# hiimmuc/SpeakerVerification

Hardware: AMD Instinct MI355X
Metric: embeddings/sec (2 s @16 kHz) (higher is better)
Workload: dtype bf16

## Files before the change

### speakerverification_amd/csrc/res2net.hip

```cpp
#include "common.h"
#include "kernels.h"

namespace svhip {

namespace {

#ifdef SVHIP_GEMM_DEBUG
constexpr bool R2DBG = true;
#else
constexpr bool R2DBG = false;
#endif
constexpr int R2_TMAX = 416;

template <int CW, int MIT> struct R2Cfg {
    static constexpr int ROWB = CW * 2;
    static constexpr int NCH = ROWB / 16;
    static constexpr int NT = CW / 32;
    static constexpr int MW = 8 / NT;
    static constexpr int MI = MIT;
    static constexpr int TMAX = MW * MI * 32 < R2_TMAX ? MW * MI * 32 : R2_TMAX;
    static constexpr int U_BYTES = TMAX * ROWB;
    static constexpr int W_BYTES = CW * ROWB;
    static constexpr int LDS = U_BYTES + W_BYTES;
    static constexpr int WCH = CW * NCH / 512;
    static __device__ __forceinline__ int swz(int row) { return CW == 128 ? (row & 15) : ((row >> 1) & 7); }
};

template <int CW, int MIT>
__global__ __launch_bounds__(512, 2) void res2net_chain_kernel(Res2Params p) {
    typedef R2Cfg<CW, MIT> CF;
    constexpr int ROWB = CF::ROWB, NCH = CF::NCH, MI = CF::MI, WCH = CF::WCH;
    extern __shared__ __attribute__((aligned(16))) char smem[];
    char* U = smem;
    char* Wt = smem + CF::U_BYTES;

    const int S = p.slices > 1 ? p.slices : 1;
    const int b = (int)blockIdx.x / S, si = (int)blockIdx.x - b * S;
    const int Tg = p.T;
    const int c0 = S > 1 ? si * p.Tc : 0, c1 = S > 1 ? min(Tg, c0 + p.Tc) : Tg;
    const int l0 = S > 1 ? max(0, c0 - 7 * p.dil) : 0, l1 = S > 1 ? min(Tg, c1 + 7 * p.dil) : Tg;
    const int T = l1 - l0;
    const int tid = threadIdx.x, lane = tid & 63;
    const int wave = __builtin_amdgcn_readfirstlane(tid >> 6);
    const int wn = wave % CF::NT, wq = wave / CF::NT;
    const int fr = lane & 31, fh = lane >> 5;
    const bf16_t* __restrict__ H1 = reinterpret_cast<const bf16_t*>(p.H1) + ((int64_t)b * Tg + l0) * p.ld;
    bf16_t* __restrict__ H2 = reinterpret_cast<bf16_t*>(p.H2) + ((int64_t)b * Tg + l0) * p.ld;
    const int s0 = c0 - l0, s1 = c1 - l0;

    u32x4 wregs[WCH];
    auto wload = [&](int layer, int tap) {
        const char* wsrc = reinterpret_cast<const char*>(p.W[layer]);
        int tid_w = tid;
        asm volatile("" : "+v"(tid_w));
#pragma unroll
        for (int e = 0; e < WCH; ++e) {
            const int c = tid_w + 512 * e;
            const int n = c / NCH, ch = c % NCH;
            wregs[e] = *reinterpret_cast<const u32x4*>(wsrc + ((int64_t)n * p.Kp + tap * CW) * 2 + ch * 16);
        }
    };
    auto wstore = [&]() {
        int tid_w = tid;
        asm volatile("" : "+v"(tid_w));
#pragma unroll
        for (int e = 0; e < WCH; ++e) {
            const int c = tid_w + 512 * e;
            const int n = c / NCH, ch = c % NCH;
            *reinterpret_cast<u32x4*>(Wt + n * ROWB + ((ch ^ CF::swz(n)) << 4)) = wregs[e];
        }
    };

    wload(0, 0);
    {
        constexpr int RSTEP = 512 / NCH, RB0 = 4;
        const int row0 = tid / NCH, ch0 = tid % NCH;
        const uint32_t goff0 = ((uint32_t)row0 * (uint32_t)p.ld + (uint32_t)ch0 * 8u) * 2u;
        const uint32_t gstep = (uint32_t)RSTEP * (uint32_t)p.ld * 2u;
        const char* h1b = reinterpret_cast<const char*>(H1);
        char* h2b = reinterpret_cast<char*>(H2);
        for (int it0 = 0; it0 * RSTEP < T; it0 += RB0) {
            u32x4 cc0[RB0], cc1[RB0];
#pragma unroll
            for (int k = 0; k < RB0; ++k)
                if (row0 + (it0 + k) * RSTEP < T) {
                    cc0[k] = __builtin_nontemporal_load(reinterpret_cast<const u32x4*>(h1b + goff0 + (uint32_t)(it0 + k) * gstep));
                    cc1[k] = __builtin_nontemporal_load(reinterpret_cast<const u32x4*>(h1b + CW * 2 + goff0 + (uint32_t)(it0 + k) * gstep));
                }
#pragma unroll
            for (int k = 0; k < RB0; ++k) {
                const int row = row0 + (it0 + k) * RSTEP;
                if (row < T) {
                    if (row >= s0 && row < s1) *reinterpret_cast<u32x4*>(h2b + goff0 + (uint32_t)(it0 + k) * gstep) = cc0[k];
                    *reinterpret_cast<u32x4*>(U + row * ROWB + ((ch0 ^ CF::swz(row)) << 4)) = cc1[k];
                }
            }
        }
    }
    wstore();
    __syncthreads();
    const bool stamp = R2DBG && (p.debug & 64) && p.ts && tid == 0;
    unsigned long long tprev = 0;
    if (R2DBG && (p.debug & 64) && p.ts) tprev = __builtin_readcyclecounter();
    if (stamp) p.ts[(size_t)blockIdx.x * 32 + 3] = tprev;
#define R2_STAMP(stage, k) if (R2DBG && (p.debug & 64) && p.ts) { const unsigned long long t_ = __builtin_readcyclecounter(); if (stamp) p.ts[(size_t)blockIdx.x * 32 + (stage) * 4 + (k)] = t_ - tprev; tprev = t_; }

    for (int s = 1; s < 8; ++s) {
        const int layer = s - 1;
        f32x16 acc[MI];
        float zero = 0.0f;
        asm volatile("" : "+v"(zero));
#pragma unroll
        for (int i = 0; i < MI; ++i)
#pragma unroll
            for (int r = 0; r < 16; ++r) acc[i][r] = zero;

        constexpr int RSTEP = 512 / NCH;
        constexpr int RB = 7;
        constexpr int NPRE = (CF::TMAX / RSTEP + RB - 1) / RB * RB;
        const bool noglob = R2DBG && (p.debug & 1);

        u32x4 cpre[NPRE];
        for (int tap = 0; tap < 3; ++tap) {
            if (tap == 2 && s < 7 && !noglob) {
                int tid_p = tid;
                asm volatile("" : "+v"(tid_p));
                const int row0 = tid_p / NCH, ch0 = tid_p % NCH;
                const char* h1s = reinterpret_cast<const char*>(H1) + (s + 1) * CW * 2;
#pragma unroll
                for (int k = 0; k < NPRE; ++k) {
                    const int rowc = min(row0 + k * RSTEP, T - 1);
                    cpre[k] = __builtin_nontemporal_load(reinterpret_cast<const u32x4*>(h1s + ((uint32_t)rowc * (uint32_t)p.ld + (uint32_t)ch0 * 8u) * 2u));
                }
            }
            const bool more = !(s == 7 && tap == 2);
            if (more && !(R2DBG && (p.debug & 4))) { if (tap < 2) wload(layer, tap + 1); else wload(layer + 1, 0); }
            const int delta = (tap - 1) * p.dil;
            int fh_t = fh, fr_t = fr;
            asm volatile("" : "+v"(fh_t), "+v"(fr_t));
            int rbase[MI], rsw[MI];
#pragma unroll
            for (int i = 0; i < MI; ++i) {
                const int t = (wq + CF::MW * i) * 32 + fr_t + delta;
                const int row = min(max(reflect_idx(l0 + t, Tg) - l0, 0), T - 1);
                rbase[i] = row * ROWB;
                rsw[i] = CF::swz(row);
            }
            const int wrow = (wn * 32 + fr_t);
            const int wbase = wrow * ROWB, wsw = CF::swz(wrow);
            if (!(R2DBG && (p.debug & 2))) {
                constexpr int NK = CW / 16;
#pragma unroll
                for (int kk = 0; kk < NK; ++kk) {
                    const int ch = 2 * kk + fh_t;
                    const bf16x8 wf = *reinterpret_cast<const bf16x8*>(Wt + wbase + ((ch ^ wsw) << 4));
                    bf16x8 xf[MI];
#pragma unroll
                    for (int i = 0; i < MI; ++i) xf[i] = *reinterpret_cast<const bf16x8*>(U + rbase[i] + ((ch ^ rsw[i]) << 4));
#pragma unroll
                    for (int i = 0; i < MI; ++i) acc[i] = __builtin_amdgcn_mfma_f32_32x32x16_bf16(wf, xf[i], acc[i], 0, 0, 0);
                }
            }
            __syncthreads();
            if (tap < 2) { if (!(R2DBG && (p.debug & 4))) wstore(); __syncthreads(); }
        }

        R2_STAMP(s, 0)
        int fh_e = fh, fr_e = fr;
        asm volatile("" : "+v"(fh_e), "+v"(fr_e));
        if (!(R2DBG && (p.debug & 8)))
#pragma unroll
        for (int g = 0; g < 4; ++g) {
            const int n = wn * 32 + 8 * g + 4 * fh_e;
            const f32x4 b4 = *reinterpret_cast<const f32x4*>(p.bias[layer] + n);
            const f32x4 sc4 = *reinterpret_cast<const f32x4*>(p.scale[layer] + n);
            const f32x4 sh4 = *reinterpret_cast<const f32x4*>(p.shift[layer] + n);
#pragma unroll
            for (int i = 0; i < MI; ++i) {
                const int t = (wq + CF::MW * i) * 32 + fr_e;
                if (t < T) {
                    typedef bf16_t bf16x4 __attribute__((ext_vector_type(4)));
                    bf16x4 o;
#pragma unroll
                    for (int e = 0; e < 4; ++e) o[e] = static_cast<bf16_t>(fmaf(fmaxf(acc[i][4 * g + e] + b4[e], 0.0f), sc4[e], sh4[e]));
                    const int c8 = n >> 2;
                    *reinterpret_cast<bf16x4*>(U + t * ROWB + ((((c8 >> 1) ^ CF::swz(t)) << 4) | ((c8 & 1) << 3))) = o;
                }
            }
        }
        if (s < 7 && !(R2DBG && (p.debug & 4))) wstore();
        __syncthreads();
        R2_STAMP(s, 1)

        if (R2DBG && (p.debug & 32)) {
            for (int c = tid; c < T * NCH; c += 512) {
                const int row = c / NCH, ch = c % NCH;
                char* up = U + row * ROWB + ((ch ^ CF::swz(row)) << 4);
                const bf16x8 y = *reinterpret_cast<const bf16x8*>(up);
                if (row >= s0 && row < s1) *reinterpret_cast<bf16x8*>(H2 + (int64_t)row * p.ld + s * CW + ch * 8) = y;
                if (s < 7) {
                    const bf16x8 cn = *reinterpret_cast<const bf16x8*>(H1 + (int64_t)row * p.ld + (s + 1) * CW + ch * 8);
                    bf16x8 u;
#pragma unroll
                    for (int e = 0; e < 8; ++e) u[e] = static_cast<bf16_t>(static_cast<float>(y[e]) + static_cast<float>(cn[e]));
                    *reinterpret_cast<bf16x8*>(up) = u;
                }
            }
        } else {
            int tid_r = tid;
            asm volatile("" : "+v"(tid_r));
            const int row0 = tid_r / NCH, ch0 = tid_r % NCH;
            const uint32_t goff0 = ((uint32_t)row0 * (uint32_t)p.ld + (uint32_t)ch0 * 8u) * 2u;
            const uint32_t gstep = (uint32_t)RSTEP * (uint32_t)p.ld * 2u;
            char* h2s = reinterpret_cast<char*>(H2) + s * CW * 2;
#pragma unroll
            for (int g = 0; g < NPRE / RB; ++g) {
                const int it0 = g * RB;
                if (it0 * RSTEP < T) {
#pragma unroll
                    for (int k = 0; k < RB; ++k) {
                        const int row = row0 + (it0 + k) * RSTEP;
                        if (row < T) {
                            char* up = U + row * ROWB + ((ch0 ^ CF::swz(row)) << 4);
                            const bf16x8 y = *reinterpret_cast<const bf16x8*>(up);
                            if (!noglob && row >= s0 && row < s1) *reinterpret_cast<bf16x8*>(h2s + goff0 + (uint32_t)(it0 + k) * gstep) = y;
                            if (s < 7 && !noglob) {
                                const bf16x8 cv = __builtin_bit_cast(bf16x8, cpre[it0 + k]);
                                bf16x8 u;
#pragma unroll
                                for (int e = 0; e < 8; ++e) u[e] = static_cast<bf16_t>(static_cast<float>(y[e]) + static_cast<float>(cv[e]));
                                *reinterpret_cast<bf16x8*>(up) = u;
                            }
                        }
                    }
                }
            }
        }
        __syncthreads();
        R2_STAMP(s, 2)
    }
#undef R2_STAMP
}

template <int CW, int MIT>
hipError_t launch_cw(const Res2Params& p, int grid, hipStream_t stream) {
    static DeviceOnce attr;
    constexpr int lds = R2Cfg<CW, MIT>::LDS;
    if (hipError_t e = set_max_dynamic_lds(attr, reinterpret_cast<const void*>(res2net_chain_kernel<CW, MIT>), lds)) return e;
    hipLaunchKernelGGL((res2net_chain_kernel<CW, MIT>), dim3(grid), dim3(512), lds, stream, p);
    return hipGetLastError();
}

}

int res2net_chain_slices(int B, int C, int T, int dil, int num_cu) {
    const int cw = C / 8;
    const int tmax_s = cw == 128 ? R2Cfg<128, 3>::TMAX : R2Cfg<64, 2>::TMAX;
    int best = 1;
    for (int S = 2; S <= 7; ++S) {
        const int tc = (T + S - 1) / S;
        if ((int64_t)S * B > (int64_t)num_cu) break;
        if (tc + 14 * dil <= tmax_s && tc > 14 * dil) best = S;
    }
    return best;
}

bool res2net_chain_supported(int C, int T, int dil, int Kp) {
    const int cw = C / 8;
    return (cw == 64 || cw == 128) && T <= R2_TMAX && T > 2 * dil && Kp == 3 * cw;
}

hipError_t launch_res2net_chain(const Res2Params& p_in, int B, int C, hipStream_t stream) {
    if (!res2net_chain_supported(C, p_in.T, p_in.dil, p_in.Kp) || B <= 0 || p_in.ld % 8 != 0) return hipErrorInvalidValue;
    Res2Params p = p_in;
    if (p.slices > 1) {
        const int tmax_s = C / 8 == 128 ? R2Cfg<128, 3>::TMAX : R2Cfg<64, 2>::TMAX;
        while (p.slices > 1) {
            p.Tc = (p.T + p.slices - 1) / p.slices;
            if (p.Tc + 14 * p.dil <= tmax_s && p.Tc > 14 * p.dil) break;
            --p.slices;
        }
        if (p.slices > 1) return C / 8 == 128 ? launch_cw<128, 3>(p, B * p.slices, stream) : launch_cw<64, 2>(p, B * p.slices, stream);
    }
    p.slices = 1;
    return C / 8 == 128 ? launch_cw<128, 7>(p, B, stream) : launch_cw<64, 4>(p, B, stream);
}

}
```

Baseline: 60290.

## Add dedicated loader waves to res2net chain kernel for global I/O overlap

For the CW=128 non-sliced path, the kernel now launches 768 threads: 8 waves run the MFMA matmuls and 4 extra loader waves prefetch the next slice input from H1, add it into the LDS tile, and write finished outputs to H2. Global loads and stores are meant to overlap with compute instead of sitting serially between layers. The loader waves stay in lockstep with the compute waves through matching __syncthreads counts. The price is more threads per block, a lower occupancy bound of 3, and fragile barrier pairing between the two branches.

```diff
diff --git a/speakerverification_amd/csrc/res2net.hip b/speakerverification_amd/csrc/res2net.hip
--- a/speakerverification_amd/csrc/res2net.hip
+++ b/speakerverification_amd/csrc/res2net.hip
@@ -26,10 +26,10 @@
     static __device__ __forceinline__ int swz(int row) { return CW == 128 ? (row & 15) : ((row >> 1) & 7); }
 };
 
-template <int CW, int MIT>
-__global__ __launch_bounds__(512, 2) void res2net_chain_kernel(Res2Params p) {
+template <int CW, int MIT, bool LW>
+__global__ __launch_bounds__(LW ? 768 : 512, LW ? 3 : 2) void res2net_chain_kernel(Res2Params p) {
     typedef R2Cfg<CW, MIT> CF;
-    constexpr int ROWB = CF::ROWB, NCH = CF::NCH, MI = CF::MI, WCH = CF::WCH;
+    constexpr int ROWB = CF::ROWB, NCH = CF::NCH, MI = CF::MI;
     extern __shared__ __attribute__((aligned(16))) char smem[];
     char* U = smem;
     char* Wt = smem + CF::U_BYTES;
@@ -42,36 +42,68 @@
     const int T = l1 - l0;
     const int tid = threadIdx.x, lane = tid & 63;
     const int wave = __builtin_amdgcn_readfirstlane(tid >> 6);
+    const bool mat = !LW || wave < 8;
     const int wn = wave % CF::NT, wq = wave / CF::NT;
     const int fr = lane & 31, fh = lane >> 5;
     const bf16_t* __restrict__ H1 = reinterpret_cast<const bf16_t*>(p.H1) + ((int64_t)b * Tg + l0) * p.ld;
     bf16_t* __restrict__ H2 = reinterpret_cast<bf16_t*>(p.H2) + ((int64_t)b * Tg + l0) * p.ld;
     const int s0 = c0 - l0, s1 = c1 - l0;
 
+    constexpr int WT = 512;
+    constexpr int WCH = CW * NCH / WT;
+    const int wtid = tid;
     u32x4 wregs[WCH];
     auto wload = [&](int layer, int tap) {
         const char* wsrc = reinterpret_cast<const char*>(p.W[layer]);
-        int tid_w = tid;
+        int tid_w = wtid;
         asm volatile("" : "+v"(tid_w));
 #pragma unroll
         for (int e = 0; e < WCH; ++e) {
-            const int c = tid_w + 512 * e;
+            const int c = tid_w + WT * e;
             const int n = c / NCH, ch = c % NCH;
             wregs[e] = *reinterpret_cast<const u32x4*>(wsrc + ((int64_t)n * p.Kp + tap * CW) * 2 + ch * 16);
         }
     };
     auto wstore = [&]() {
-        int tid_w = tid;
+        int tid_w = wtid;
         asm volatile("" : "+v"(tid_w));
 #pragma unroll
         for (int e = 0; e < WCH; ++e) {
-            const int c = tid_w + 512 * e;
+            const int c = tid_w + WT * e;
             const int n = c / NCH, ch = c % NCH;
             *reinterpret_cast<u32x4*>(Wt + n * ROWB + ((ch ^ CF::swz(n)) << 4)) = wregs[e];
         }
     };
 
-    wload(0, 0);
+    constexpr int LROWS = 256 / NCH;
+    constexpr int NLC = LW ? (CF::TMAX + LROWS - 1) / LROWS : 1;
+    static_assert(!LW || (CW == 128 && NLC * LROWS <= CF::TMAX), "the loader rows cover U exactly");
+    u32x4 creg[NLC];
+    const int lt = LW ? tid - 512 : 0;
+    const int lrow0 = lt / NCH, lch = lt % NCH;
+    auto cload = [&](int sn) {
+        const char* h1s = reinterpret_cast<const char*>(H1) + sn * CW * 2;
+        int r0 = lrow0, c16 = lch * 16;
+        asm volatile("" : "+v"(r0), "+v"(c16));
+#pragma unroll
+        for (int k = 0; k < NLC; ++k) {
+            const int rowc = min(r0 + k * LROWS, T - 1);
+            creg[k] = __builtin_nontemporal_load(reinterpret_cast<const u32x4*>(h1s + ((uint32_t)rowc * (uint32_t)p.ld * 2u + (uint32_t)c16)));
+        }
+    };
+    auto ystore = [&](int sy) {
+        char* h2s = reinterpret_cast<char*>(H2) + sy * CW * 2;
+        int r0 = lrow0, c16 = lch * 16;
+        asm volatile("" : "+v"(r0), "+v"(c16));
+#pragma unroll
+        for (int k = 0; k < NLC; ++k) {
+            const int row = r0 + k * LROWS;
+            if (row < T) *reinterpret_cast<u32x4*>(h2s + ((uint32_t)row * (uint32_t)p.ld * 2u + (uint32_t)c16)) = creg[k];
+        }
+    };
+
+    if (mat) wload(0, 0);
+    if (mat)
     {
         constexpr int RSTEP = 512 / NCH, RB0 = 4;
         const int row0 = tid / NCH, ch0 = tid % NCH;
@@ -97,13 +129,122 @@
             }
         }
     }
-    wstore();
+    if (mat) wstore();
     __syncthreads();
     const bool stamp = R2DBG && (p.debug & 64) && p.ts && tid == 0;
     unsigned long long tprev = 0;
     if (R2DBG && (p.debug & 64) && p.ts) tprev = __builtin_readcyclecounter();
     if (stamp) p.ts[(size_t)blockIdx.x * 32 + 3] = tprev;
 #define R2_STAMP(stage, k) if (R2DBG && (p.debug & 64) && p.ts) { const unsigned long long t_ = __builtin_readcyclecounter(); if (stamp) p.ts[(size_t)blockIdx.x * 32 + (stage) * 4 + (k)] = t_ - tprev; tprev = t_; }
+
+    if constexpr (LW) {
+        const bool noglob = R2DBG && (p.debug & 1);
+        const bool noslab = R2DBG && (p.debug & 4);
+        if (mat) {
+            for (int s = 1; s < 8; ++s) {
+                const int layer = s - 1;
+                f32x16 acc[MI];
+                float zero = 0.0f;
+                asm volatile("" : "+v"(zero));
+#pragma unroll
+                for (int i = 0; i < MI; ++i)
+#pragma unroll
+                    for (int r = 0; r < 16; ++r) acc[i][r] = zero;
+                for (int tap = 0; tap < 3; ++tap) {
+                    if (!(s == 7 && tap == 2) && !noslab) { if (tap < 2) wload(layer, tap + 1); else wload(layer + 1, 0); }
+                    const int delta = (tap - 1) * p.dil;
+                    int fh_t = fh, fr_t = fr;
+                    asm volatile("" : "+v"(fh_t), "+v"(fr_t));
+                    int rbase[MI], rsw[MI];
+#pragma unroll
+                    for (int i = 0; i < MI; ++i) {
+                        const int t = (wq + CF::MW * i) * 32 + fr_t + delta;
+                        const int row = min(max(reflect_idx(t, Tg), 0), T - 1);
+                        rbase[i] = row * ROWB;
+                        rsw[i] = CF::swz(row);
+                    }
+                    const int wrow = (wn * 32 + fr_t);
+                    const int wbase = wrow * ROWB, wsw = CF::swz(wrow);
+                    if (!(R2DBG && (p.debug & 2))) {
+                        constexpr int NK = CW / 16;
+#pragma unroll
+                        for (int kk = 0; kk < NK; ++kk) {
+                            const int ch = 2 * kk + fh_t;
+                            const bf16x8 wf = *reinterpret_cast<const bf16x8*>(Wt + wbase + ((ch ^ wsw) << 4));
+                            bf16x8 xf[MI];
+#pragma unroll
+                            for (int i = 0; i < MI; ++i) xf[i] = *reinterpret_cast<const bf16x8*>(U + rbase[i] + ((ch ^ rsw[i]) << 4));
+#pragma unroll
+                            for (int i = 0; i < MI; ++i) acc[i] = __builtin_amdgcn_mfma_f32_32x32x16_bf16(wf, xf[i], acc[i], 0, 0, 0);
+                        }
+                    }
+                    __syncthreads();
+                    if (tap < 2) { if (!noslab) wstore(); __syncthreads(); }
+                }
+                R2_STAMP(s, 0)
+                int fh_e = fh, fr_e = fr;
+                asm volatile("" : "+v"(fh_e), "+v"(fr_e));
+                if (!(R2DBG && (p.debug & 8)))
+#pragma unroll
+                for (int g = 0; g < 4; ++g) {
+                    const int n = wn * 32 + 8 * g + 4 * fh_e;
+                    const f32x4 b4 = *reinterpret_cast<const f32x4*>(p.bias[layer] + n);
+                    const f32x4 sc4 = *reinterpret_cast<const f32x4*>(p.scale[layer] + n);
+                    const f32x4 sh4 = *reinterpret_cast<const f32x4*>(p.shift[layer] + n);
+#pragma unroll
+                    for (int i = 0; i < MI; ++i) {
+                        const int t = (wq + CF::MW * i) * 32 + fr_e;
+                        if (t < T) {
+                            typedef bf16_t bf16x4 __attribute__((ext_vector_type(4)));
+                            bf16x4 o;
+#pragma unroll
+                            for (int e = 0; e < 4; ++e) o[e] = static_cast<bf16_t>(fmaf(fmaxf(acc[i][4 * g + e] + b4[e], 0.0f), sc4[e], sh4[e]));
+                            const int c8 = n >> 2;
+                            *reinterpret_cast<bf16x4*>(U + t * ROWB + ((((c8 >> 1) ^ CF::swz(t)) << 4) | ((c8 & 1) << 3))) = o;
+                        }
+                    }
+                }
+                if (s < 7 && !noslab) wstore();
+                __syncthreads();
+                R2_STAMP(s, 1)
+                __syncthreads();
+                R2_STAMP(s, 2)
+            }
+        } else {
+            for (int s = 1; s < 8; ++s) {
+                if (s > 1 && !noglob) ystore(s - 1);
+                if (s < 7 && !noglob) cload(s + 1);
+                __syncthreads();
+                R2_STAMP(s, 0)
+#pragma unroll
+                for (int k = 0; k < 5; ++k) __syncthreads();
+                if (R2DBG && (p.debug & 64) && p.ts && lt == 0) {
+                    const unsigned long long t0 = __builtin_readcyclecounter();
+                    asm volatile("s_waitcnt vmcnt(0)" ::: "memory");
+                    p.ts[(size_t)blockIdx.x * 32 + s * 4 + 3] = __builtin_readcyclecounter() - t0;
+                }
+                int r0 = lrow0, ch0 = lch;
+                asm volatile("" : "+v"(r0), "+v"(ch0));
+#pragma unroll
+                for (int k = 0; k < NLC; ++k) {
+                    const int row = r0 + k * LROWS;
+                    char* up = U + row * ROWB + ((ch0 ^ CF::swz(row)) << 4);
+                    const bf16x8 y = *reinterpret_cast<const bf16x8*>(up);
+                    if (s < 7 && !noglob) {
+                        const bf16x8 cv = __builtin_bit_cast(bf16x8, creg[k]);
+                        bf16x8 u;
+#pragma unroll
+                        for (int e = 0; e < 8; ++e) u[e] = static_cast<bf16_t>(static_cast<float>(y[e]) + static_cast<float>(cv[e]));
+                        *reinterpret_cast<bf16x8*>(up) = u;
+                    }
+                    creg[k] = __builtin_bit_cast(u32x4, y);
+                }
+                __syncthreads();
+            }
+            if (!noglob) ystore(7);
+        }
+        return;
+    }
 
     for (int s = 1; s < 8; ++s) {
         const int layer = s - 1;
@@ -242,12 +383,12 @@
 #undef R2_STAMP
 }
 
-template <int CW, int MIT>
+template <int CW, int MIT, bool LW = false>
 hipError_t launch_cw(const Res2Params& p, int grid, hipStream_t stream) {
     static DeviceOnce attr;
     constexpr int lds = R2Cfg<CW, MIT>::LDS;
-    if (hipError_t e = set_max_dynamic_lds(attr, reinterpret_cast<const void*>(res2net_chain_kernel<CW, MIT>), lds)) return e;
-    hipLaunchKernelGGL((res2net_chain_kernel<CW, MIT>), dim3(grid), dim3(512), lds, stream, p);
+    if (hipError_t e = set_max_dynamic_lds(attr, reinterpret_cast<const void*>(res2net_chain_kernel<CW, MIT, LW>), lds)) return e;
+    hipLaunchKernelGGL((res2net_chain_kernel<CW, MIT, LW>), dim3(grid), dim3(LW ? 768 : 512), lds, stream, p);
     return hipGetLastError();
 }
 
@@ -283,7 +424,8 @@
         if (p.slices > 1) return C / 8 == 128 ? launch_cw<128, 3>(p, B * p.slices, stream) : launch_cw<64, 2>(p, B * p.slices, stream);
     }
     p.slices = 1;
-    return C / 8 == 128 ? launch_cw<128, 7>(p, B, stream) : launch_cw<64, 4>(p, B, stream);
-}
-
-}
+    if (C / 8 == 64) return launch_cw<64, 4>(p, B, stream);
+    return (p.debug & 128) ? launch_cw<128, 7>(p, B, stream) : launch_cw<128, 7, true>(p, B, stream);
+}
+
+}
```

After: 60440 (median of 6 runs). About the same (+0.3%).
